# jaidevshriram/loma-nerf

Hardware: AMD Instinct MI355X
Metric: ray-samples/sec fwd+bwd, 4096 rays×64 samples, 1/2/4/8 MI355X (higher is better)
Workload: dtype f32; 1 GPU; cfg3: 4096 rays x 64 samples per GPU, PE F=5, MLP 33->256x7->4, fp32; rays_per_gpu=4096, samples=64, layers=8, width=256, parallelism=dp1, optimizer=adam lr 0.0005 on device (train_nerf.py:133-161), in the step, input=rays: sampling, dists and positional encoding on the GPU

## Files before the change

loma-nerf_amd/csrc/lnerf_dw16.hip:

```cpp
#include "lnerf_internal.h"

namespace lnerf {

namespace {

typedef float fx4 __attribute__((ext_vector_type(4)));
typedef float fx16 __attribute__((ext_vector_type(16)));
typedef __bf16 bf8 __attribute__((ext_vector_type(8)));
typedef __bf16 bf4 __attribute__((ext_vector_type(4)));
typedef _Float16 hf8 __attribute__((ext_vector_type(8)));
typedef _Float16 hf4 __attribute__((ext_vector_type(4)));

#ifndef LNERF_DW16_SPLIT_LATE
#define LNERF_DW16_SPLIT_LATE 1
#endif
#ifndef LNERF_DW16_DEPTH
#define LNERF_DW16_DEPTH 3
#endif

#ifndef LNERF_DW16_XROW
#define LNERF_DW16_XROW 1
#endif

#ifndef LNERF_DW16_WAVES
#define LNERF_DW16_WAVES 8
#endif
constexpr int kWavesDw = LNERF_DW16_WAVES;
static_assert(kWavesDw == 16 || kWavesDw == 8 || kWavesDw == 4, "dW workgroups of 16, 8 or 4 waves");
constexpr int kThreads = 64 * kWavesDw;
// ... 51 lines not shown
__device__ __forceinline__ RowMap row_map(int kt, int nt) {
    RowMap m;
    const int t = threadIdx.x, u = t & 127;
    m.lane = 4 * u;
    m.hstride = 512;
    m.rowo = 16 * ((t >> 6) & 1) + 4 * (t & 3);
    m.isamp = (t & 63) >> 2;
    const int w2 = wave_id() >> 1;
#pragma unroll
    for (int i = 0; i < kRounds; ++i) {
        const int tl = kTileGroups * (i % kRPO) + w2;
        m.ok[i] = tl < (i < kRPO ? kt : nt);
        m.tile[i] = m.ok[i] ? tl : 0;
    }
    return m;
}

__device__ __forceinline__ int image_row(int i, const RowMap& m) {
    return (i < kRPO ? 0 : 256) + 32 * (kTileGroups * (i % kRPO) + (threadIdx.x >> 7)) + m.rowo;
}

struct Loads {
    fx4 v[kRounds];
    unsigned e;
};

__device__ __forceinline__ void sample_shifts(unsigned e, int E, int& ea, int& eg) {
    const int xa = sexp_xa(e), xg = sexp_xg(e);
    if (xa == -128 || xg == -128) {
        ea = xa < -126 ? 0 : xa;
        eg = xg == -128 ? 0 : xg;
        return;
    }
    if (xa == kSexpNonFinite) {
        eg = xg;
        ea = E - xg;
        return;
    }
    const int d = xa + xg - E;
    ea = xa - (d >> 1);
    eg = xg - ((d + 1) >> 1);
}

template <bool A24>
__device__ __forceinline__ void issue_loads(const float* A, const float* G, const unsigned* se, int kt,
                                            int nt, const RowMap& m, int hb, int hb_end, Loads& L) {
    const bool in = hb < hb_end;
    const int hbc = in ? hb : max(0, hb_end - 1);
    L.e = se[hbc * 16 + m.isamp];
    const int blk = hbc >> 1, half = hbc & 1;
    const float* pg = G + (size_t)blk * nt * 1024 + half * m.hstride;
    if constexpr (A24) {
        const unsigned char* pa = (const unsigned char*)A + ((size_t)blk * kt * 3072 + half * 1536 + 12 * (threadIdx.x & 127));
#pragma unroll
        for (int i = 0; i < kRPO; ++i) {
            const unsigned* q = (const unsigned*)(pa + m.tile[i] * 3072);
            L.v[i] = fx4{__builtin_bit_cast(float, __builtin_nontemporal_load(q)),
                         __builtin_bit_cast(float, __builtin_nontemporal_load(q + 1)),
                         __builtin_bit_cast(float, __builtin_nontemporal_load(q + 2)), 0.0f};
        }
    } else {
        const float* pa = A + (size_t)blk * kt * 1024 + half * m.hstride;
#pragma unroll
        for (int i = 0; i < kRPO; ++i) L.v[i] = __builtin_nontemporal_load((const fx4*)(pa + m.tile[i] * 1024 + m.lane));
    }
#pragma unroll
    for (int i = kRPO; i < kRounds; ++i) L.v[i] = __builtin_nontemporal_load((const fx4*)(pg + m.tile[i] * 1024 + m.lane));
}

__device__ __forceinline__ fx4 decode_a24(const fx4& raw) {
    typedef unsigned ux4 __attribute__((ext_vector_type(4)));
    const ux4 d = __builtin_bit_cast(ux4, raw);
    const unsigned d0 = d[0], d1 = d[1], d2 = d[2];
    const unsigned m0 = d0 & 0xFFFFFFu;
    const unsigned m1 = __builtin_amdgcn_alignbit(d1, d0, 24) & 0xFFFFFFu;
    const unsigned m2 = __builtin_amdgcn_alignbit(d2, d1, 16) & 0xFFFFFFu;
    const unsigned m3 = d2 >> 8;
    constexpr float kMagic = 12582912.0f;
    return fx4{__builtin_bit_cast(float, 0x4B000000u | m0) - kMagic, __builtin_bit_cast(float, 0x4B000000u | m1) - kMagic,
               __builtin_bit_cast(float, 0x4B000000u | m2) - kMagic, __builtin_bit_cast(float, 0x4B000000u | m3) - kMagic};
}

__device__ __forceinline__ void split4(const fx4& x, bf4& h, bf4& m, bf4& lo) {
#pragma unroll
    for (int e = 0; e < 4; ++e) {
        const __bf16 hh = (__bf16)x[e];
        const float r = x[e] - (float)hh;
        const __bf16 mm = (__bf16)r;
        h[e] = hh;
        m[e] = mm;
        lo[e] = (__bf16)(r - (float)mm);
    }
}


template <int PL>
__device__ __forceinline__ void write_planes_row(const fx4& v, int i, unsigned char* img, float sa, float sg,
                                                 const RowMap& m) {
    unsigned char* p = img + m.isamp * kImgRow + 8 * ((image_row(i, m) >> 2) ^ swz(m.isamp));
    const float sc = i < kRPO ? sa : sg;
    if constexpr (PL == 2) {
        typedef unsigned u2 __attribute__((ext_vector_type(2)));
        unsigned h0, l0, h1, l1;
        split_h2(v[0], v[1], sc, h0, l0);
        split_h2(v[2], v[3], sc, h1, l1);
        *(u2*)(p) = u2{h0, h1};
        *(u2*)(p + kPlaneBytes) = u2{l0, l1};
    } else if constexpr (PL == 1) {
        const fx4 x = v * sc;
        *(bf4*)(p) = bf4{(__bf16)x[0], (__bf16)x[1], (__bf16)x[2], (__bf16)x[3]};
    } else {
        bf4 h, m, lo;
        split4(v * sc, h, m, lo);
        *(bf4*)(p) = h;
        *(bf4*)(p + kPlaneBytes) = m;
        *(bf4*)(p + 2 * kPlaneBytes) = lo;
    }
}

__device__ __forceinline__ bool xrow(unsigned e, int E) {
    const int xa = sexp_xa(e), xg = sexp_xg(e);
    const int d = xa + xg - E;
    return xa > -127 && xg > -127 && (d < 0 || d > sexp_dmax(e));
}

template <int PL>
__device__ __forceinline__ void sample_scales(unsigned e, int E, float& sa, float& sg) {
    int ea, eg;
    sample_shifts(e, E, ea, eg);
    if constexpr (a24k(PL)) {
        const int xa = sexp_xa(e);
        ea = xa == -128 ? 0 : ea - (xa == kSexpNonFinite ? 0 : xa) - 8;
    }
    sa = __builtin_ldexpf(1.0f, ea);
    sg = __builtin_ldexpf(1.0f, eg);
    if constexpr (PL == 2 && LNERF_DW16_XROW) {
        const bool x = xrow(e, E);
        sa = x ? 0.0f : sa;
        sg = x ? 0.0f : sg;
    }
}

template <int PL>
__device__ __forceinline__ fx4 round_values(const Loads& L, int i) {
    if constexpr (a24k(PL)) {
        if (i >= kRPO) return L.v[i];
        fx4 v = decode_a24(L.v[i]);
        const bool marked = sexp_xa(L.e) == kSexpNonFinite;
        if (__builtin_expect(__builtin_amdgcn_ballot_w64(marked) != 0, 0)) {
#pragma unroll
            for (int j = 0; j < 4; ++j)
                if (marked && __builtin_fabsf(v[j]) >= 4194304.0f) v[j] = __builtin_nanf("");
            asm volatile("" : "+v"(v));
        }
        return v;
    }
    return L.v[i];
}

template <int PL>
__device__ __forceinline__ void write_planes(const Loads& L, unsigned char* img, int E, const RowMap& m) {
    float sa, sg;
    sample_scales<PL>(L.e, E, sa, sg);
#pragma unroll
    for (int i = 0; i < kRounds; ++i) write_planes_row<PL>(round_values<PL>(L, i), i, img, sa, sg, m);
}

__device__ __forceinline__ fx16 mfma32(const bf8& a, const bf8& b, fx16 c) {
    return __builtin_amdgcn_mfma_f32_32x32x16_bf16(a, b, c, 0, 0, 0);
}
__device__ __forceinline__ fx16 mfma32h(const bf8& a, const bf8& b, fx16 c) {
    return __builtin_amdgcn_mfma_f32_32x32x16_f16(__builtin_bit_cast(hf8, a), __builtin_bit_cast(hf8, b), c, 0, 0,
                                                  0);
}

typedef short s4 __attribute__((ext_vector_type(4)));

__device__ __forceinline__ bf8 read_frag(unsigned char* addr) {
    typedef __attribute__((address_space(3))) s4* lp;
    const s4 a = __builtin_amdgcn_ds_read_tr16_b64_v4i16((lp)(__attribute__((address_space(3))) void*)addr);
    const s4 b = __builtin_amdgcn_ds_read_tr16_b64_v4i16(
        (lp)(__attribute__((address_space(3))) void*)(addr + 4 * kImgRow));
    typedef short s8 __attribute__((ext_vector_type(8)));
    return __builtin_bit_cast(bf8, s8{a[0], a[1], a[2], a[3], b[0], b[1], b[2], b[3]});
}

__device__ __forceinline__ int frag_off(int f0) {
    const int l = threadIdx.x & 63;
    const int row = 8 * (l >> 5) + ((l >> 2) & 3);
    const int quad = (f0 >> 2) + 4 * ((l >> 4) & 1) + (l & 3);
    return row * kImgRow + 8 * (quad ^ swz(row));
}

template <int PL>
__device__ __forceinline__ fx16 mma_tile(const bf8 (&ap)[nplanes(PL)], const bf8 (&gp)[nplanes(PL)], fx16 c) {
    if constexpr (PL == 2) {
        c = mfma32h(ap[0], gp[1], c);
        c = mfma32h(ap[1], gp[0], c);
        c = mfma32h(ap[0], gp[0], c);
    } else if constexpr (PL == 1) {
        c = mfma32(ap[0], gp[0], c);
    } else {
        c = mfma32(ap[0], gp[2], c);
        c = mfma32(ap[1], gp[1], c);
        c = mfma32(ap[2], gp[0], c);
        c = mfma32(ap[1], gp[0], c);
        c = mfma32(ap[0], gp[1], c);
        c = mfma32(ap[0], gp[0], c);
    }
    return c;
}

#ifndef LNERF_DW16_PMAJOR
#define LNERF_DW16_PMAJOR 1
#endif
// ... 2 lines not shown
                                        fx16 (&acc)[TI][TJ], int j) {
    if constexpr (!LNERF_DW16_PMAJOR) {
#pragma unroll
        for (int i = 0; i < TI; ++i) acc[i][j] = mma_tile<PL>(ap[i], gp, acc[i][j]);
    } else if constexpr (PL == 2) {
#pragma unroll
        for (int i = 0; i < TI; ++i) acc[i][j] = mfma32h(ap[i][0], gp[1], acc[i][j]);
#pragma unroll
        for (int i = 0; i < TI; ++i) acc[i][j] = mfma32h(ap[i][1], gp[0], acc[i][j]);
#pragma unroll
        for (int i = 0; i < TI; ++i) acc[i][j] = mfma32h(ap[i][0], gp[0], acc[i][j]);
    } else if constexpr (PL == 1) {
#pragma unroll
        for (int i = 0; i < TI; ++i) acc[i][j] = mfma32(ap[i][0], gp[0], acc[i][j]);
    } else {
        constexpr int pa[6] = {0, 1, 2, 1, 0, 0}, pg[6] = {2, 1, 0, 0, 1, 0};
#pragma unroll
        for (int k = 0; k < 6; ++k)
#pragma unroll
            for (int i = 0; i < TI; ++i) acc[i][j] = mfma32(ap[i][pa[k]], gp[pg[k]], acc[i][j]);
    }
}

template <int PL, int TI, int TJ, bool ACTIVE, bool FULL>
__device__ __forceinline__ void block_mma(const unsigned char* img, int a0, int g0, fx16 (&acc)[TI][TJ],
                                          const Loads& nl, unsigned char* nxt, const RowMap& m, int E,
                                          bool live = true) {
    float sa, sg;
    sample_scales<PL>(nl.e, E, sa, sg);
    sa = live ? sa : 0.0f;
    sg = live ? sg : 0.0f;
    const unsigned char* fl = img;
    constexpr int NP = nplanes(PL);
    bf8 ap[TI][NP];
    if constexpr (ACTIVE) {
#pragma unroll
        for (int i = 0; i < TI; ++i)
#pragma unroll
            for (int p = 0; p < NP; ++p) ap[i][p] = read_frag((unsigned char*)fl + p * kPlaneBytes + frag_off(a0 + 32 * i));
    }
    constexpr int RPS = (kWavesDw == 8 || TJ >= kRounds) ? 1 : (kRounds + TJ - 1) / TJ;
    constexpr int NR = (kRounds + RPS - 1) / RPS;
    constexpr int NK = NR > TJ ? NR : TJ;
    auto split = [&](int k) {
#pragma unroll
        for (int r = 0; r < RPS; ++r) {
            const int i = k * RPS + r;
            if (i < kRounds && (FULL || m.ok[i])) write_planes_row<PL>(round_values<PL>(nl, i), i, nxt, sa, sg, m);
        }
    };
#pragma unroll
    for (int k = 0; k < NK; ++k) {
        if (!LNERF_DW16_SPLIT_LATE) split(k);
        if constexpr (ACTIVE) {
            if (k < TJ) {
                const int j = k < TJ ? k : 0;
                bf8 gp[NP];
#pragma unroll
                for (int p = 0; p < NP; ++p) gp[p] = read_frag((unsigned char*)fl + p * kPlaneBytes + frag_off(256 + g0 + 32 * j));
                mma_col<PL, TI, TJ>(ap, gp, acc, j);
            }
        }
        if (LNERF_DW16_SPLIT_LATE) split(k);
    }
}

template <int PL, int TI, int TJ, bool ACTIVE, bool FULL, int I>
__device__ __forceinline__ void hb_step3(const float* A, const float* G, const unsigned* se, int kt, int nt,
                                         const RowMap& m, int hb, int hb0, int hb1, int a0, int g0,
                                         fx16 (&acc)[TI][TJ], Loads& L0, Loads& L1, Loads& L2, fx4 (&dbs)[kRPO],
                                         unsigned char* lds, int E, bool& xany) {
    constexpr int kIB = image_bytes<PL>();
    Loads& fr = I == 0 ? L0 : I == 1 ? L1 : L2;
    const Loads& nx = I == 0 ? L1 : I == 1 ? L2 : L0;
    issue_loads<a24k(PL)>(A, G, se, kt, nt, m, hb + 3, hb1, fr);
    if (hb + 1 < hb1) {
#pragma unroll
        for (int i = 0; i < kRPO; ++i) dbs[i] += nx.v[kRPO + i];
    }
    const int cur = (hb - hb0) & 1;
    block_mma<PL, TI, TJ, ACTIVE, FULL>(lds + cur * kIB, a0, g0, acc, nx, lds + (cur ^ 1) * kIB, m, E, hb + 1 < hb1);
    if constexpr (PL == 2 && LNERF_DW16_XROW) xany |= hb + 1 < hb1 && xrow(nx.e, E);
    __syncthreads();
}

template <int PL, int TI, int TJ, bool ACTIVE, bool FULL>
__device__ __forceinline__ void hb_loop3(const float* A, const float* G, const unsigned* se, int kt, int nt,
                                         const RowMap& m, int hb0, int hb1, int a0, int g0, fx16 (&acc)[TI][TJ],
                                         Loads& L0, Loads& L1, Loads& L2, fx4 (&dbs)[kRPO], unsigned char* lds,
                                         int E, bool& xany) {
    for (int hb = hb0; hb < hb1; hb += 3) {
        hb_step3<PL, TI, TJ, ACTIVE, FULL, 0>(A, G, se, kt, nt, m, hb, hb0, hb1, a0, g0, acc, L0, L1, L2, dbs, lds, E, xany);
        hb_step3<PL, TI, TJ, ACTIVE, FULL, 1>(A, G, se, kt, nt, m, hb + 1, hb0, hb1, a0, g0, acc, L0, L1, L2, dbs, lds, E, xany);
        hb_step3<PL, TI, TJ, ACTIVE, FULL, 2>(A, G, se, kt, nt, m, hb + 2, hb0, hb1, a0, g0, acc, L0, L1, L2, dbs, lds, E, xany);
    }
}

template <int PL, int TI, int TJ, bool ACTIVE, bool FULL, int I>
__device__ __forceinline__ void hb_step2(const float* A, const float* G, const unsigned* se, int kt, int nt,
                                         const RowMap& m, int hb, int hb0, int hb1, int a0, int g0,
                                         fx16 (&acc)[TI][TJ], Loads& L0, Loads& L1, fx4 (&dbs)[kRPO],
                                         unsigned char* lds, int E, bool& xany) {
    constexpr int kIB = image_bytes<PL>();
    Loads& fr = I == 0 ? L0 : L1;
    const Loads& nx = I == 0 ? L1 : L0;
    issue_loads<a24k(PL)>(A, G, se, kt, nt, m, hb + 2, hb1, fr);
    if (hb + 1 < hb1) {
#pragma unroll
        for (int i = 0; i < kRPO; ++i) dbs[i] += nx.v[kRPO + i];
    }
    const int cur = (hb - hb0) & 1;
    block_mma<PL, TI, TJ, ACTIVE, FULL>(lds + cur * kIB, a0, g0, acc, nx, lds + (cur ^ 1) * kIB, m, E, hb + 1 < hb1);
    if constexpr (PL == 2 && LNERF_DW16_XROW) xany |= hb + 1 < hb1 && xrow(nx.e, E);
    __syncthreads();
}

template <int PL, int TI, int TJ, bool ACTIVE, bool FULL>
__device__ __forceinline__ void hb_loop2(const float* A, const float* G, const unsigned* se, int kt, int nt,
                                         const RowMap& m, int hb0, int hb1, int a0, int g0, fx16 (&acc)[TI][TJ],
                                         Loads& L0, Loads& L1, fx4 (&dbs)[kRPO], unsigned char* lds, int E,
                                         bool& xany) {
    for (int hb = hb0; hb < hb1; hb += 2) {
        hb_step2<PL, TI, TJ, ACTIVE, FULL, 0>(A, G, se, kt, nt, m, hb, hb0, hb1, a0, g0, acc, L0, L1, dbs, lds, E, xany);
        hb_step2<PL, TI, TJ, ACTIVE, FULL, 1>(A, G, se, kt, nt, m, hb + 1, hb0, hb1, a0, g0, acc, L0, L1, dbs, lds, E, xany);
    }
}

template <bool A24>
__device__ __forceinline__ void gather_loads(const float* A, const float* G, const unsigned* se, int kt, int nt,
                                             const RowMap& m, int p, Loads& L) {
    const int pc = p < 0 ? 0 : p;
    L.e = se[pc];
    const int hb = pc >> 4, blk = hb >> 1, half = hb & 1;
    const int u = ((int)threadIdx.x & 127 & ~0x3C) | ((pc & 15) << 2);
    const float* pg = G + (size_t)blk * nt * 1024 + half * 512 + 4 * u;
    if constexpr (A24) {
        const unsigned char* pa = (const unsigned char*)A + ((size_t)blk * kt * 3072 + half * 1536 + 12 * u);
#pragma unroll
        for (int i = 0; i < kRPO; ++i) {
            const unsigned* q = (const unsigned*)(pa + m.tile[i] * 3072);
            L.v[i] = fx4{__builtin_bit_cast(float, q[0]), __builtin_bit_cast(float, q[1]),
                         __builtin_bit_cast(float, q[2]), 0.0f};
        }
    } else {
        const float* pa = A + (size_t)blk * kt * 1024 + half * 512 + 4 * u;
#pragma unroll
        for (int i = 0; i < kRPO; ++i) L.v[i] = *(const fx4*)(pa + m.tile[i] * 1024);
    }
#pragma unroll
    for (int i = kRPO; i < kRounds; ++i) L.v[i] = *(const fx4*)(pg + m.tile[i] * 1024);
}

template <int PL, int TI, int TJ>
__device__ __forceinline__ void mma_block(const unsigned char* img, int a0, int g0, fx16 (&acc)[TI][TJ]) {
    constexpr int NP = nplanes(PL);
    bf8 ap[TI][NP];
#pragma unroll
    for (int i = 0; i < TI; ++i)
#pragma unroll
        for (int p = 0; p < NP; ++p) ap[i][p] = read_frag((unsigned char*)img + p * kPlaneBytes + frag_off(a0 + 32 * i));
#pragma unroll
    for (int j = 0; j < TJ; ++j) {
        bf8 gp[NP];
#pragma unroll
        for (int p = 0; p < NP; ++p) gp[p] = read_frag((unsigned char*)img + p * kPlaneBytes + frag_off(256 + g0 + 32 * j));
// ... 58 lines not shown
                ring[(mine + r) % kXrowRing] = base + k * kThreads + tid;
            }
        }
        tail = off;
        __syncthreads();
        const bool last = base + 4 * kThreads >= p1;
        const int ng = last ? (tail - head + 15) / 16 : (tail - head) / 16;
        if (ng > 0) {
            auto pos = [&](int gi) {
                const int at = head + 16 * gi + m.isamp;
                return at < tail ? ring[at % kXrowRing] : -1;
            };
            int pc = pos(0);
            Loads Lc;
            gather_loads<a24k(PX)>(A, G, se, KT, NT, m, pc, Lc);
            for (int gi = 0; gi < ng; ++gi) {
                const int pn = gi + 1 < ng ? pos(gi + 1) : -1;
                Loads Ln;
                if (gi + 1 < ng) gather_loads<a24k(PX)>(A, G, se, KT, NT, m, pn, Ln);
                float sa, sg;
                sample_scales<PX>(Lc.e, E, sa, sg);
                sa = pc < 0 ? 0.0f : sa;
                sg = pc < 0 ? 0.0f : sg;
#pragma unroll
                for (int i = 0; i < kRounds; ++i)
                    if (m.ok[i]) write_planes_row<PX>(round_values<PX>(Lc, i), i, lds, sa, sg, m);
                __syncthreads();
                if (active) mma_block<PX, TI, TJ>(lds, a0, g0, acc);
                __syncthreads();
                Lc = Ln;
                pc = pn;
            }
            head = head + 16 * ng < tail ? head + 16 * ng : tail;
        }
    }
    return int2{tail, ntail};
}

template <int PL, int TI, int TJ>
__device__ __forceinline__ void dw_split(const Dw16Args& a, int l, int sp, unsigned char* lds) {
    const int tid = threadIdx.x, lane = tid & 63, wave = wave_id();
    const int KT = a.kt[l], NT = a.nt[l];
    const int nbg = (NT + TJ - 1) / TJ, nblk = ((KT + TI - 1) / TI) * nbg;
    const bool active = wave < nblk;
    const int a0 = active ? (wave / nbg) * 32 * TI : 0, g0 = active ? (wave % nbg) * 32 * TJ : 0;
    const int hbs = 2 * a.blocks, splits = a.splits[l];
    const int per = (hbs + splits - 1) / splits;
    const int hb0 = min(hbs, sp * per), hb1 = min(hbs, hb0 + per);

    fx16 acc[TI][TJ];
#pragma unroll
    for (int i = 0; i < TI; ++i)
#pragma unroll
        for (int j = 0; j < TJ; ++j) acc[i][j] = fx16{0, 0, 0, 0, 0, 0, 0, 0, 0, 0, 0, 0, 0, 0, 0, 0};
    fx4 dbs[kRPO];
#pragma unroll
    for (int i = 0; i < kRPO; ++i) dbs[i] = fx4{0.0f, 0.0f, 0.0f, 0.0f};

    const float* A = a.act + a.a_off[l];
    const float* G = a.grad + a.g_off[l];
    const RowMap m = row_map(KT, NT);
    const unsigned* se = a.sexp + (size_t)l * a.rpad;
    const int E = a.eshift[l];
    const bool full = KT == 8 && NT == 8;
#if LNERF_DW16_DEPTH == 2
    Loads L0, L1;
    bool xany = false;
    issue_loads<a24k(PL)>(A, G, se, KT, NT, m, hb0, hb1, L0);
    issue_loads<a24k(PL)>(A, G, se, KT, NT, m, hb0 + 1, hb1, L1);
    if (hb0 < hb1) {
#pragma unroll
        for (int i = 0; i < kRPO; ++i) dbs[i] += L0.v[kRPO + i];
        write_planes<PL>(L0, lds, E, m);
        if constexpr (PL == 2 && LNERF_DW16_XROW) xany = xrow(L0.e, E);
    }
    __syncthreads();
    if (active && full) hb_loop2<PL, TI, TJ, true, true>(A, G, se, KT, NT, m, hb0, hb1, a0, g0, acc, L0, L1, dbs, lds, E, xany);
    else if (active) hb_loop2<PL, TI, TJ, true, false>(A, G, se, KT, NT, m, hb0, hb1, a0, g0, acc, L0, L1, dbs, lds, E, xany);
    else if (full) hb_loop2<PL, TI, TJ, false, true>(A, G, se, KT, NT, m, hb0, hb1, a0, g0, acc, L0, L1, dbs, lds, E, xany);
    else hb_loop2<PL, TI, TJ, false, false>(A, G, se, KT, NT, m, hb0, hb1, a0, g0, acc, L0, L1, dbs, lds, E, xany);
#else
    Loads L0, L1, L2;
    bool xany = false;
    issue_loads<a24k(PL)>(A, G, se, KT, NT, m, hb0, hb1, L0);
    issue_loads<a24k(PL)>(A, G, se, KT, NT, m, hb0 + 1, hb1, L1);
    issue_loads<a24k(PL)>(A, G, se, KT, NT, m, hb0 + 2, hb1, L2);
    if (hb0 < hb1) {
#pragma unroll
        for (int i = 0; i < kRPO; ++i) dbs[i] += L0.v[kRPO + i];
        write_planes<PL>(L0, lds, E, m);
        if constexpr (PL == 2 && LNERF_DW16_XROW) xany = xrow(L0.e, E);
    }
    __syncthreads();
    if (active && full) hb_loop3<PL, TI, TJ, true, true>(A, G, se, KT, NT, m, hb0, hb1, a0, g0, acc, L0, L1, L2, dbs, lds, E, xany);
    else if (active) hb_loop3<PL, TI, TJ, true, false>(A, G, se, KT, NT, m, hb0, hb1, a0, g0, acc, L0, L1, L2, dbs, lds, E, xany);
    else if (full) hb_loop3<PL, TI, TJ, false, true>(A, G, se, KT, NT, m, hb0, hb1, a0, g0, acc, L0, L1, L2, dbs, lds, E, xany);
    else hb_loop3<PL, TI, TJ, false, false>(A, G, se, KT, NT, m, hb0, hb1, a0, g0, acc, L0, L1, L2, dbs, lds, E, xany);
#endif

    if constexpr (PL == 2 && LNERF_DW16_XROW) {
        const int2 nx = xrow_pass<TI, TJ>(A, G, se, KT, NT, m, hb0, hb1, a0, g0, active, acc, lds, E, xany);
        if (threadIdx.x == 0 && a.xcount) {
            a.xcount[2 * blockIdx.x] = nx.x;
            a.xcount[2 * blockIdx.x + 1] = nx.y;
        }
    } else {
        if (threadIdx.x == 0 && a.xcount) a.xcount[2 * blockIdx.x] = a.xcount[2 * blockIdx.x + 1] = 0;
    }

    if (active) {
        const int ncol = NT * 32, h = lane >> 5;
        float* part = a.dw_part + a.dwp_off[l] + (size_t)sp * (KT * 32) * ncol;
#pragma unroll
        for (int i = 0; i < TI; ++i)
#pragma unroll
            for (int j = 0; j < TJ; ++j) {
                const int kb = a0 + 32 * i, jb = g0 + 32 * j;
                if (kb < KT * 32 && jb < ncol) {
#pragma unroll
                    for (int r = 0; r < 16; ++r) {
                        const int k = kb + (r & 3) + 8 * (r >> 2) + 4 * h;
// ... 20 lines not shown
}

__host__ __device__ __forceinline__ int dw_shape(int kt, int nt) {
    auto fits = [&](int ti, int tj) { return ((kt + ti - 1) / ti) * ((nt + tj - 1) / tj) <= kWavesDw; };
    if (kWavesDw == 8) {
        if (fits(1, 1)) return 0;
        if (fits(1, 2)) return 1;
        return 2;
    }
    if (kWavesDw == 16) {
        if (fits(1, 1)) return 0;
        if (fits(1, 2)) return 1;
        if (fits(2, 1)) return 3;
        return 4;
    }
    if (fits(1, 1)) return 0;
    if (fits(2, 1)) return 3;
    if (fits(1, 2)) return 1;
    if (fits(2, 2)) return 4;
    return 5;
}

template <int PL>
constexpr int dw_lds_bytes() {
    constexpr int main = 2 * image_bytes<PL>();
    constexpr int xr = PL == 2 && LNERF_DW16_XROW ? image_bytes<kXrowPL>() + (kXrowRing + 9 * kWavesDw) * 4 : 0;
    return main > xr ? main : xr;
}

template <int PL>
__global__ void __launch_bounds__(kThreads, 1) __attribute__((amdgpu_waves_per_eu(kWavesDw / 4, kWavesDw / 4)))
dw16_kernel(Dw16Args a) {
    __shared__ __attribute__((aligned(16))) unsigned char lds[dw_lds_bytes<PL>()];
    if (a.gate && *a.gate == 0) return;
    int li = 0;
    while (li + 1 < a.nl && (int)blockIdx.x >= a.wg_off[li + 1]) ++li;
    const int l = a.lid[li], sp = blockIdx.x - a.wg_off[li];
    if constexpr (kWavesDw == 8) {
        switch (dw_shape(a.kt[l], a.nt[l])) {
            case 0: dw_split<PL, 1, 1>(a, l, sp, lds); break;
            case 1: dw_split<PL, 1, 2>(a, l, sp, lds); break;
            default: dw_split<PL, 2, 4>(a, l, sp, lds); break;
        }
    } else if constexpr (kWavesDw == 16) {
        switch (dw_shape(a.kt[l], a.nt[l])) {
            case 0: dw_split<PL, 1, 1>(a, l, sp, lds); break;
            case 1: dw_split<PL, 1, 2>(a, l, sp, lds); break;
            case 3: dw_split<PL, 2, 1>(a, l, sp, lds); break;
            default: dw_split<PL, 2, 2>(a, l, sp, lds); break;
        }
    } else {
        switch (dw_shape(a.kt[l], a.nt[l])) {
            case 0: dw_split<PL, 1, 1>(a, l, sp, lds); break;
            case 3: dw_split<PL, 2, 1>(a, l, sp, lds); break;
            case 1: dw_split<PL, 1, 2>(a, l, sp, lds); break;
            case 4: dw_split<PL, 2, 2>(a, l, sp, lds); break;
// ... 22 lines not shown
            for (int w = 1; w < 16; ++w) r = min(r, ired[w]);
            eshift[blockIdx.x] = r == (1 << 20) ? 0 : r;
        }
        return;
    }
    float s = 0.0f;
    if (t < 256)
        for (int i = t; i < nwg; i += 256) s += loss_part[i];
    red[t] = s;
    __syncthreads();
    for (int w = 128; w > 0; w >>= 1) {
        if (t < w) red[t] = red[t] + red[t + w];
        __syncthreads();
    }
    if (t == 0) {
        *total = red[0];
        if (out_loss) *out_loss = red[0];
    }
}

}

unsigned dw16_build_knobs() {
    return (LNERF_DW16_SPLIT_LATE != 1 ? kKnobDwSplitLate : 0u) | (LNERF_DW16_DEPTH != 3 ? kKnobDwDepth : 0u) |
           (LNERF_DW16_SWZ != 1 ? kKnobDwSwz : 0u) | (LNERF_A24 != 1 ? kKnobA24 : 0u) |
           (LNERF_DW16_XROW != 1 ? kKnobDwXrow : 0u) |
           (LNERF_DW16_WAVES != 8 || !LNERF_DW16_PMAJOR ? kKnobDwWaves : 0u);
}

void dw16_launch(const FusedPlan& p, hipStream_t s) {
    Dw16Args a{};
    for (int l = 0; l < p.L; ++l) {
        a.kt[l] = p.kt[l];
        a.nt[l] = p.nt[l];
        a.a_off[l] = (l == 0) ? p.x_off : p.act_off[l - 1];
        a.g_off[l] = p.grad_off[l];
        a.splits[l] = p.dw_splits[l];
        a.dwp_off[l] = p.dwp_off[l];
        a.dbp_off[l] = p.dbp_off[l];
        a.lid[l] = l;
        a.wg_off[l] = p.dw_split_off[l];
    }
    a.wg_off[p.L] = p.dw_grid;
    a.nl = p.L;
    a.act = p.act;
    a.grad = p.grad;
    a.blocks = p.blocks;
// ... 22 lines not shown
```

loma-nerf_amd/csrc/lnerf_internal.h:

```cpp
#pragma once

#include <hip/hip_runtime.h>
#include <stddef.h>
#include <stdint.h>

#include "lnerf.h"
#include "lnerf_marshal.h"

namespace lnerf {

constexpr int kWmaxParts = 32;
constexpr int kHeadCols = 16;
constexpr int kDefaultDwGrid = 512;
__host__ __device__ constexpr int default_dw_grid(long long samples) {
    return samples / 128 >= kDefaultDwGrid ? kDefaultDwGrid : samples / 128 <= 256 ? 256 : (int)(samples / 128);
}
constexpr int kXrowD0 = 12;
constexpr int kXrowLast = 127;
__host__ __device__ constexpr int sexp_xa(unsigned e) { return (int)(signed char)(e & 0xFFu); }
__host__ __device__ constexpr int sexp_xg(unsigned e) { return (int)(signed char)((e >> 16) & 0xFFu); }
__host__ __device__ constexpr int sexp_dmax(unsigned e) { return (int)(signed char)(e >> 24); }

__device__ __forceinline__ int fp16x3_shift(float m) {
    if (!(m > 0.0f) || !(m < __builtin_inff())) return 0;
// ... 6 lines not shown
__device__ __forceinline__ void split_h2(float x0, float x1, float sc, unsigned& hi, unsigned& lo) {
    typedef _Float16 h2 __attribute__((ext_vector_type(2)));
    const _Float16 h0 = (_Float16)__builtin_fmaf(x0, sc, 0.0f);
    const _Float16 h1 = (_Float16)__builtin_fmaf(x1, sc, 0.0f);
    const _Float16 l0 = (_Float16)__builtin_fmaf(x0, sc, -(float)h0);
    const _Float16 l1 = (_Float16)__builtin_fmaf(x1, sc, -(float)h1);
    hi = __builtin_bit_cast(unsigned, (h2){h0, h1});
    lo = __builtin_bit_cast(unsigned, (h2){l0, l1});
}

#ifndef LNERF_A24
#define LNERF_A24 1
#endif
__host__ __device__ constexpr bool a24_slabs(int PL) { return PL == 2 && LNERF_A24 != 0; }
constexpr int kSexpNonFinite = -127;
__host__ __device__ constexpr int a_tile_floats(int PL) { return a24_slabs(PL) ? 768 : 1024; }

enum : unsigned {
    kKnobK16FullDma = 1u << 0, kKnobK16KDist = 1u << 1, kKnobK16SplitAt = 1u << 2, kKnobK16Sched = 1u << 3,
    kKnobK16Prio = 1u << 4, kKnobK16Spread = 1u << 5, kKnobProf = 1u << 6, kKnobA24 = 1u << 7,
    kKnobK16Only = 1u << 8, kKnobDwSplitLate = 1u << 9, kKnobDwDepth = 1u << 10, kKnobDwSwz = 1u << 11,
    kKnobK16Pin = 1u << 12, kKnobK16FdSrc = 1u << 13, kKnobKrStagger = 1u << 15, kKnobDwXrow = 1u << 17,
    kKnobGuard = 1u << 25, kKnobK16G2 = 1u << 26, kKnobKrSched = 1u << 18, kKnobDwWaves = 1u << 14, kKnobKrDist = 1u << 19, kKnobPeDoubling = 1u << 20, kKnobK16OneChunk = 1u << 22, kKnobK16WaveComp = 1u << 23, kKnobK16EpiFma = 1u << 24,
};
unsigned k16_build_knobs();
unsigned dw16_build_knobs();
unsigned kr_build_knobs();

__host__ __device__ inline double ray_depth(int j, int S, float near_t, float far_t) {
    if (S <= 1) return (double)near_t;
    if (j == S - 1) return (double)far_t;
    return (double)j * (((double)far_t - (double)near_t) / (double)(S - 1)) + (double)near_t;
}
__host__ __device__ inline float ray_delta(int j, int S, float near_t, float far_t) {
    if (j >= S - 1) return 1e8f;
    return (float)(ray_depth(j + 1, S, near_t, far_t) - ray_depth(j, S, near_t, far_t));
}
__host__ __device__ inline double ray_point(const float* ray6, int c, int j, int S, float near_t,
                                            float far_t) {
    return (double)ray6[c] + (double)ray6[3 + c] * ray_depth(j, S, near_t, far_t);
}


struct LgBuffers {
    const float* X;
    const float* W;
// ... 123 lines not shown
```

Measured before the change: 118.5 million ray-samples/s.

## Precompute per-sample scale table in LDS and interleave dW16 loads with MFMA

The dW16 weight-gradient kernel now precomputes per-sample scale factors into an LDS table in chunks, so the main loop no longer loads and decodes the exponent word every step. Global loads for future blocks are split by round and issued between MFMA columns. A24 activations are read with a single 96-bit buffer load. The G fragment reads are prefetched one column ahead around the fp16 MFMAs, and the LDS addressing is simplified with XOR tile offsets. The aim is to hide load latency and cut scalar and address overhead in the hot loop, at the cost of more LDS, an extra sync per chunk and more register pressure.

```diff
diff --git a/loma-nerf_amd/csrc/lnerf_dw16.hip b/loma-nerf_amd/csrc/lnerf_dw16.hip
--- a/loma-nerf_amd/csrc/lnerf_dw16.hip
+++ b/loma-nerf_amd/csrc/lnerf_dw16.hip
@@ -5,6 +5,7 @@
 namespace {
 
 typedef float fx4 __attribute__((ext_vector_type(4)));
+typedef float fx3 __attribute__((ext_vector_type(3)));
 typedef float fx16 __attribute__((ext_vector_type(16)));
 typedef __bf16 bf8 __attribute__((ext_vector_type(8)));
 typedef __bf16 bf4 __attribute__((ext_vector_type(4)));
@@ -102,55 +103,50 @@
 
 struct Loads {
     fx4 v[kRounds];
+    fx3 a24[kRPO];
     unsigned e;
 };
 
 __device__ __forceinline__ void sample_shifts(unsigned e, int E, int& ea, int& eg) {
     const int xa = sexp_xa(e), xg = sexp_xg(e);
-    if (xa == -128 || xg == -128) {
-        ea = xa < -126 ? 0 : xa;
-        eg = xg == -128 ? 0 : xg;
-        return;
-    }
-    if (xa == kSexpNonFinite) {
-        eg = xg;
-        ea = E - xg;
-        return;
-    }
+    const bool zero = xa == -128 || xg == -128, nonfin = xa == kSexpNonFinite;
     const int d = xa + xg - E;
-    ea = xa - (d >> 1);
-    eg = xg - ((d + 1) >> 1);
-}
-
+    ea = zero ? (xa < -126 ? 0 : xa) : nonfin ? E - xg : xa - (d >> 1);
+    eg = zero ? (xg == -128 ? 0 : xg) : nonfin ? xg : xg - ((d + 1) >> 1);
+}
+
+constexpr int kAllRounds = (1 << kRounds) - 1;
 template <bool A24>
-__device__ __forceinline__ void issue_loads(const float* A, const float* G, const unsigned* se, int kt,
-                                            int nt, const RowMap& m, int hb, int hb_end, Loads& L) {
+__device__ __forceinline__ void issue_loads(const float* A, const float* G, int kt, int nt, const RowMap& m,
+                                            int hb, int hb_end, Loads& L, int rounds = kAllRounds) {
     const bool in = hb < hb_end;
     const int hbc = in ? hb : max(0, hb_end - 1);
-    L.e = se[hbc * 16 + m.isamp];
     const int blk = hbc >> 1, half = hbc & 1;
     const float* pg = G + (size_t)blk * nt * 1024 + half * m.hstride;
-    if constexpr (A24) {
-        const unsigned char* pa = (const unsigned char*)A + ((size_t)blk * kt * 3072 + half * 1536 + 12 * (threadIdx.x & 127));
+    if (!(rounds & ((1 << kRPO) - 1))) {
+    } else if constexpr (A24) {
+        const unsigned char* pa = (const unsigned char*)A + ((size_t)blk * kt * 3072 + half * 1536);
+        const __amdgpu_buffer_rsrc_t rs =
+            __builtin_amdgcn_make_buffer_rsrc((void*)pa, 0, kt * 3072 - 1536, 0x00020000);
 #pragma unroll
         for (int i = 0; i < kRPO; ++i) {
-            const unsigned* q = (const unsigned*)(pa + m.tile[i] * 3072);
-            L.v[i] = fx4{__builtin_bit_cast(float, __builtin_nontemporal_load(q)),
-                         __builtin_bit_cast(float, __builtin_nontemporal_load(q + 1)),
-                         __builtin_bit_cast(float, __builtin_nontemporal_load(q + 2)), 0.0f};
+            if (rounds >> i & 1)
+                L.a24[i] = __builtin_bit_cast(fx3, __builtin_amdgcn_raw_buffer_load_b96(rs, 3 * m.lane, m.tile[i] * 3072, 2));
         }
     } else {
         const float* pa = A + (size_t)blk * kt * 1024 + half * m.hstride;
 #pragma unroll
-        for (int i = 0; i < kRPO; ++i) L.v[i] = __builtin_nontemporal_load((const fx4*)(pa + m.tile[i] * 1024 + m.lane));
-    }
-#pragma unroll
-    for (int i = kRPO; i < kRounds; ++i) L.v[i] = __builtin_nontemporal_load((const fx4*)(pg + m.tile[i] * 1024 + m.lane));
-}
-
-__device__ __forceinline__ fx4 decode_a24(const fx4& raw) {
-    typedef unsigned ux4 __attribute__((ext_vector_type(4)));
-    const ux4 d = __builtin_bit_cast(ux4, raw);
+        for (int i = 0; i < kRPO; ++i)
+            if (rounds >> i & 1) L.v[i] = __builtin_nontemporal_load((const fx4*)(pa + m.tile[i] * 1024 + m.lane));
+    }
+#pragma unroll
+    for (int i = kRPO; i < kRounds; ++i)
+        if (rounds >> i & 1) L.v[i] = __builtin_nontemporal_load((const fx4*)(pg + m.tile[i] * 1024 + m.lane));
+}
+
+__device__ __forceinline__ fx4 decode_a24(const fx3& raw) {
+    typedef unsigned ux3 __attribute__((ext_vector_type(3)));
+    const ux3 d = __builtin_bit_cast(ux3, raw);
     const unsigned d0 = d[0], d1 = d[1], d2 = d[2];
     const unsigned m0 = d0 & 0xFFFFFFu;
     const unsigned m1 = __builtin_amdgcn_alignbit(d1, d0, 24) & 0xFFFFFFu;
@@ -177,7 +173,11 @@
 template <int PL>
 __device__ __forceinline__ void write_planes_row(const fx4& v, int i, unsigned char* img, float sa, float sg,
                                                  const RowMap& m) {
-    unsigned char* p = img + m.isamp * kImgRow + 8 * ((image_row(i, m) >> 2) ^ swz(m.isamp));
+    constexpr bool kRoundConst = kRPO == 1 || kTileGroups % 4 == 0;
+    const int qround = (i < kRPO ? 0 : 64) + 8 * kTileGroups * (i % kRPO);
+    unsigned char* p = kRoundConst
+        ? img + m.isamp * kImgRow + 8 * (((image_row(0, m) >> 2) ^ swz(m.isamp))) + 8 * qround
+        : img + m.isamp * kImgRow + 8 * ((image_row(i, m) >> 2) ^ swz(m.isamp));
     const float sc = i < kRPO ? sa : sg;
     if constexpr (PL == 2) {
         typedef unsigned u2 __attribute__((ext_vector_type(2)));
@@ -221,13 +221,14 @@
     }
 }
 
-template <int PL>
-__device__ __forceinline__ fx4 round_values(const Loads& L, int i) {
+__device__ __forceinline__ bool any_marked(bool marked) { return __builtin_amdgcn_ballot_w64(marked) != 0; }
+
+template <int PL>
+__device__ __forceinline__ fx4 round_values(const Loads& L, int i, bool marked, bool anym) {
     if constexpr (a24k(PL)) {
         if (i >= kRPO) return L.v[i];
-        fx4 v = decode_a24(L.v[i]);
-        const bool marked = sexp_xa(L.e) == kSexpNonFinite;
-        if (__builtin_expect(__builtin_amdgcn_ballot_w64(marked) != 0, 0)) {
+        fx4 v = decode_a24(L.a24[i]);
+        if (__builtin_expect(anym, 0)) {
 #pragma unroll
             for (int j = 0; j < 4; ++j)
                 if (marked && __builtin_fabsf(v[j]) >= 4194304.0f) v[j] = __builtin_nanf("");
@@ -238,12 +239,40 @@
     return L.v[i];
 }
 
-template <int PL>
-__device__ __forceinline__ void write_planes(const Loads& L, unsigned char* img, int E, const RowMap& m) {
+struct SampleScale {
     float sa, sg;
-    sample_scales<PL>(L.e, E, sa, sg);
-#pragma unroll
-    for (int i = 0; i < kRounds; ++i) write_planes_row<PL>(round_values<PL>(L, i), i, img, sa, sg, m);
+    bool marked;
+};
+__device__ __forceinline__ SampleScale decode_scale(const float2& t) {
+    const unsigned b = __builtin_bit_cast(unsigned, t.x);
+    return SampleScale{__builtin_bit_cast(float, b & 0x7FFFFFFFu), t.y, (b >> 31) != 0};
+}
+
+constexpr int kTabPast = 4;
+template <int PL>
+__device__ __forceinline__ bool fill_scales(float2* tab, const unsigned* se, int E, int c0, int c1) {
+    bool x = false;
+    const int n = (c1 - c0 + kTabPast) * 16, nin = (c1 - c0) * 16, last = max(0, c1 - 1) * 16;
+    for (int i = threadIdx.x; i < n; i += kThreads) {
+        const bool in = i < nin;
+        const unsigned e = se[in ? c0 * 16 + i : last + (i & 15)];
+        float sa, sg;
+        sample_scales<PL>(e, E, sa, sg);
+        unsigned ba = in ? __builtin_bit_cast(unsigned, sa) : 0u;
+        if constexpr (a24k(PL)) ba |= sexp_xa(e) == kSexpNonFinite ? 0x80000000u : 0u;
+        if constexpr (PL == 2 && LNERF_DW16_XROW) x |= in && xrow(e, E);
+        tab[i] = float2{__builtin_bit_cast(float, ba), in ? sg : 0.0f};
+    }
+    return x;
+}
+
+template <int PL>
+__device__ __forceinline__ void write_planes(const Loads& L, unsigned char* img, const SampleScale& sc,
+                                             const RowMap& m) {
+    const bool anym = a24k(PL) && any_marked(sc.marked);
+#pragma unroll
+    for (int i = 0; i < kRounds; ++i)
+        write_planes_row<PL>(round_values<PL>(L, i, sc.marked, anym), i, img, sc.sa, sc.sg, m);
 }
 
 __device__ __forceinline__ fx16 mfma32(const bf8& a, const bf8& b, fx16 c) {
@@ -271,6 +300,12 @@
     const int quad = (f0 >> 2) + 4 * ((l >> 4) & 1) + (l & 3);
     return row * kImgRow + 8 * (quad ^ swz(row));
 }
+
+typedef __attribute__((address_space(3))) unsigned char* lds_bytes;
+__device__ __forceinline__ lds_bytes frag_tile(lds_bytes base, int t) {
+    return (lds_bytes)(unsigned long long)((unsigned)(unsigned long long)base ^ (unsigned)(t << 6));
+}
+__device__ __forceinline__ bf8 read_frag(lds_bytes addr) { return read_frag((unsigned char*)addr); }
 
 template <int PL>
 __device__ __forceinline__ fx16 mma_tile(const bf8 (&ap)[nplanes(PL)], const bf8 (&gp)[nplanes(PL)], fx16 c) {
@@ -319,23 +354,38 @@
     }
 }
 
-template <int PL, int TI, int TJ, bool ACTIVE, bool FULL>
+#ifndef LNERF_DW16_AHEAD
+#define LNERF_DW16_AHEAD 1
+#endif
+template <int PL, int TI, int TJ, bool ACTIVE, bool FULL, typename Pre, typename Mid>
 __device__ __forceinline__ void block_mma(const unsigned char* img, int a0, int g0, fx16 (&acc)[TI][TJ],
-                                          const Loads& nl, unsigned char* nxt, const RowMap& m, int E,
-                                          bool live = true) {
-    float sa, sg;
-    sample_scales<PL>(nl.e, E, sa, sg);
-    sa = live ? sa : 0.0f;
-    sg = live ? sg : 0.0f;
+                                          const Loads& nl, unsigned char* nxt, const RowMap& m, Pre&& pre,
+                                          Mid&& mid) {
     const unsigned char* fl = img;
     constexpr int NP = nplanes(PL);
+    constexpr bool AHEAD = LNERF_DW16_AHEAD != 0 && LNERF_DW16_PMAJOR != 0 && PL == 2;
     bf8 ap[TI][NP];
+    static_assert((TI & (TI - 1)) == 0 && (TJ & (TJ - 1)) == 0 && TI <= 4 && TJ <= 4, "frag_tile: aligned tile groups");
+    const lds_bytes fa = (lds_bytes)(__attribute__((address_space(3))) void*)(fl + frag_off(a0));
+    const lds_bytes fg = (lds_bytes)(__attribute__((address_space(3))) void*)(fl + frag_off(256 + g0));
+    bf8 glo, ghi;
+    auto read_g = [&](int j, int p) { return read_frag(frag_tile(fg, j) + p * kPlaneBytes); };
+    SampleScale sc;
+    if constexpr (!AHEAD) sc = pre();
     if constexpr (ACTIVE) {
 #pragma unroll
         for (int i = 0; i < TI; ++i)
 #pragma unroll
-            for (int p = 0; p < NP; ++p) ap[i][p] = read_frag((unsigned char*)fl + p * kPlaneBytes + frag_off(a0 + 32 * i));
-    }
+            for (int p = 0; p < NP; ++p) ap[i][p] = read_frag(frag_tile(fa, i) + p * kPlaneBytes);
+        if constexpr (AHEAD) {
+            glo = read_g(0, 1);
+            ghi = read_g(0, 0);
+            __builtin_amdgcn_sched_barrier(0);
+        }
+    }
+    if constexpr (AHEAD) sc = pre();
+    const float sa = sc.sa, sg = sc.sg;
+    const bool anym = a24k(PL) && any_marked(sc.marked);
     constexpr int RPS = (kWavesDw == 8 || TJ >= kRounds) ? 1 : (kRounds + TJ - 1) / TJ;
     constexpr int NR = (kRounds + RPS - 1) / RPS;
     constexpr int NK = NR > TJ ? NR : TJ;
@@ -343,7 +393,8 @@
 #pragma unroll
         for (int r = 0; r < RPS; ++r) {
             const int i = k * RPS + r;
-            if (i < kRounds && (FULL || m.ok[i])) write_planes_row<PL>(round_values<PL>(nl, i), i, nxt, sa, sg, m);
+            if (i < kRounds && (FULL || m.ok[i]))
+                write_planes_row<PL>(round_values<PL>(nl, i, sc.marked, anym), i, nxt, sa, sg, m);
         }
     };
 #pragma unroll
@@ -352,74 +403,99 @@
         if constexpr (ACTIVE) {
             if (k < TJ) {
                 const int j = k < TJ ? k : 0;
-                bf8 gp[NP];
-#pragma unroll
-                for (int p = 0; p < NP; ++p) gp[p] = read_frag((unsigned char*)fl + p * kPlaneBytes + frag_off(256 + g0 + 32 * j));
-                mma_col<PL, TI, TJ>(ap, gp, acc, j);
+                if constexpr (AHEAD) {
+#pragma unroll
+                    for (int i = 0; i < TI; ++i) acc[i][j] = mfma32h(ap[i][0], glo, acc[i][j]);
+                    if (j + 1 < TJ) {
+                        glo = read_g(j + 1, 1);
+                        __builtin_amdgcn_sched_barrier(0);
+                    }
+#pragma unroll
+                    for (int i = 0; i < TI; ++i) acc[i][j] = mfma32h(ap[i][1], ghi, acc[i][j]);
+#pragma unroll
+                    for (int i = 0; i < TI; ++i) acc[i][j] = mfma32h(ap[i][0], ghi, acc[i][j]);
+                    if (j + 1 < TJ) {
+                        ghi = read_g(j + 1, 0);
+                        __builtin_amdgcn_sched_barrier(0);
+                    }
+                } else {
+                    bf8 gp[NP];
+#pragma unroll
+                    for (int p = 0; p < NP; ++p) gp[p] = read_g(j, p);
+                    mma_col<PL, TI, TJ>(ap, gp, acc, j);
+                }
             }
         }
         if (LNERF_DW16_SPLIT_LATE) split(k);
+        if (k < NR) mid(((1 << RPS) - 1) << (k * RPS) & kAllRounds);
     }
 }
 
 template <int PL, int TI, int TJ, bool ACTIVE, bool FULL, int I>
-__device__ __forceinline__ void hb_step3(const float* A, const float* G, const unsigned* se, int kt, int nt,
+__device__ __forceinline__ void hb_step3(const float* A, const float* G, const float2* tab, int kt, int nt,
                                          const RowMap& m, int hb, int hb0, int hb1, int a0, int g0,
                                          fx16 (&acc)[TI][TJ], Loads& L0, Loads& L1, Loads& L2, fx4 (&dbs)[kRPO],
-                                         unsigned char* lds, int E, bool& xany) {
+                                         unsigned char* lds, float2& scn) {
     constexpr int kIB = image_bytes<PL>();
     Loads& fr = I == 0 ? L0 : I == 1 ? L1 : L2;
     const Loads& nx = I == 0 ? L1 : I == 1 ? L2 : L0;
-    issue_loads<a24k(PL)>(A, G, se, kt, nt, m, hb + 3, hb1, fr);
-    if (hb + 1 < hb1) {
-#pragma unroll
-        for (int i = 0; i < kRPO; ++i) dbs[i] += nx.v[kRPO + i];
-    }
+    auto pre = [&]() {
+        if (hb + 1 < hb1) {
+#pragma unroll
+            for (int i = 0; i < kRPO; ++i) dbs[i] += nx.v[kRPO + i];
+        }
+        const SampleScale sc = decode_scale(scn);
+        scn = tab[(hb + 2 - hb0) * 16];
+        return sc;
+    };
+    auto mid = [&](int rounds) { issue_loads<a24k(PL)>(A, G, kt, nt, m, hb + LNERF_DW16_DEPTH, hb1, fr, rounds); };
     const int cur = (hb - hb0) & 1;
-    block_mma<PL, TI, TJ, ACTIVE, FULL>(lds + cur * kIB, a0, g0, acc, nx, lds + (cur ^ 1) * kIB, m, E, hb + 1 < hb1);
-    if constexpr (PL == 2 && LNERF_DW16_XROW) xany |= hb + 1 < hb1 && xrow(nx.e, E);
+    block_mma<PL, TI, TJ, ACTIVE, FULL>(lds + cur * kIB, a0, g0, acc, nx, lds + (cur ^ 1) * kIB, m, pre, mid);
     __syncthreads();
 }
 
 template <int PL, int TI, int TJ, bool ACTIVE, bool FULL>
-__device__ __forceinline__ void hb_loop3(const float* A, const float* G, const unsigned* se, int kt, int nt,
+__device__ __forceinline__ void hb_loop3(const float* A, const float* G, const float2* tab, int kt, int nt,
                                          const RowMap& m, int hb0, int hb1, int a0, int g0, fx16 (&acc)[TI][TJ],
                                          Loads& L0, Loads& L1, Loads& L2, fx4 (&dbs)[kRPO], unsigned char* lds,
-                                         int E, bool& xany) {
+                                         float2& scn) {
     for (int hb = hb0; hb < hb1; hb += 3) {
-        hb_step3<PL, TI, TJ, ACTIVE, FULL, 0>(A, G, se, kt, nt, m, hb, hb0, hb1, a0, g0, acc, L0, L1, L2, dbs, lds, E, xany);
-        hb_step3<PL, TI, TJ, ACTIVE, FULL, 1>(A, G, se, kt, nt, m, hb + 1, hb0, hb1, a0, g0, acc, L0, L1, L2, dbs, lds, E, xany);
-        hb_step3<PL, TI, TJ, ACTIVE, FULL, 2>(A, G, se, kt, nt, m, hb + 2, hb0, hb1, a0, g0, acc, L0, L1, L2, dbs, lds, E, xany);
+        hb_step3<PL, TI, TJ, ACTIVE, FULL, 0>(A, G, tab, kt, nt, m, hb, hb0, hb1, a0, g0, acc, L0, L1, L2, dbs, lds, scn);
+        hb_step3<PL, TI, TJ, ACTIVE, FULL, 1>(A, G, tab, kt, nt, m, hb + 1, hb0, hb1, a0, g0, acc, L0, L1, L2, dbs, lds, scn);
+        hb_step3<PL, TI, TJ, ACTIVE, FULL, 2>(A, G, tab, kt, nt, m, hb + 2, hb0, hb1, a0, g0, acc, L0, L1, L2, dbs, lds, scn);
     }
 }
 
 template <int PL, int TI, int TJ, bool ACTIVE, bool FULL, int I>
-__device__ __forceinline__ void hb_step2(const float* A, const float* G, const unsigned* se, int kt, int nt,
+__device__ __forceinline__ void hb_step2(const float* A, const float* G, const float2* tab, int kt, int nt,
                                          const RowMap& m, int hb, int hb0, int hb1, int a0, int g0,
                                          fx16 (&acc)[TI][TJ], Loads& L0, Loads& L1, fx4 (&dbs)[kRPO],
-                                         unsigned char* lds, int E, bool& xany) {
+                                         unsigned char* lds, float2& scn) {
     constexpr int kIB = image_bytes<PL>();
     Loads& fr = I == 0 ? L0 : L1;
     const Loads& nx = I == 0 ? L1 : L0;
-    issue_loads<a24k(PL)>(A, G, se, kt, nt, m, hb + 2, hb1, fr);
-    if (hb + 1 < hb1) {
-#pragma unroll
-        for (int i = 0; i < kRPO; ++i) dbs[i] += nx.v[kRPO + i];
-    }
+    auto pre = [&]() {
+        if (hb + 1 < hb1) {
+#pragma unroll
+            for (int i = 0; i < kRPO; ++i) dbs[i] += nx.v[kRPO + i];
+        }
+        const SampleScale sc = decode_scale(scn);
+        scn = tab[(hb + 2 - hb0) * 16];
+        return sc;
+    };
+    auto mid = [&](int rounds) { issue_loads<a24k(PL)>(A, G, kt, nt, m, hb + LNERF_DW16_DEPTH, hb1, fr, rounds); };
     const int cur = (hb - hb0) & 1;
-    block_mma<PL, TI, TJ, ACTIVE, FULL>(lds + cur * kIB, a0, g0, acc, nx, lds + (cur ^ 1) * kIB, m, E, hb + 1 < hb1);
-    if constexpr (PL == 2 && LNERF_DW16_XROW) xany |= hb + 1 < hb1 && xrow(nx.e, E);
+    block_mma<PL, TI, TJ, ACTIVE, FULL>(lds + cur * kIB, a0, g0, acc, nx, lds + (cur ^ 1) * kIB, m, pre, mid);
     __syncthreads();
 }
 
 template <int PL, int TI, int TJ, bool ACTIVE, bool FULL>
-__device__ __forceinline__ void hb_loop2(const float* A, const float* G, const unsigned* se, int kt, int nt,
+__device__ __forceinline__ void hb_loop2(const float* A, const float* G, const float2* tab, int kt, int nt,
                                          const RowMap& m, int hb0, int hb1, int a0, int g0, fx16 (&acc)[TI][TJ],
-                                         Loads& L0, Loads& L1, fx4 (&dbs)[kRPO], unsigned char* lds, int E,
-                                         bool& xany) {
+                                         Loads& L0, Loads& L1, fx4 (&dbs)[kRPO], unsigned char* lds, float2& scn) {
     for (int hb = hb0; hb < hb1; hb += 2) {
-        hb_step2<PL, TI, TJ, ACTIVE, FULL, 0>(A, G, se, kt, nt, m, hb, hb0, hb1, a0, g0, acc, L0, L1, dbs, lds, E, xany);
-        hb_step2<PL, TI, TJ, ACTIVE, FULL, 1>(A, G, se, kt, nt, m, hb + 1, hb0, hb1, a0, g0, acc, L0, L1, dbs, lds, E, xany);
+        hb_step2<PL, TI, TJ, ACTIVE, FULL, 0>(A, G, tab, kt, nt, m, hb, hb0, hb1, a0, g0, acc, L0, L1, dbs, lds, scn);
+        hb_step2<PL, TI, TJ, ACTIVE, FULL, 1>(A, G, tab, kt, nt, m, hb + 1, hb0, hb1, a0, g0, acc, L0, L1, dbs, lds, scn);
     }
 }
 
@@ -436,8 +512,8 @@
 #pragma unroll
         for (int i = 0; i < kRPO; ++i) {
             const unsigned* q = (const unsigned*)(pa + m.tile[i] * 3072);
-            L.v[i] = fx4{__builtin_bit_cast(float, q[0]), __builtin_bit_cast(float, q[1]),
-                         __builtin_bit_cast(float, q[2]), 0.0f};
+            L.a24[i] = fx3{__builtin_bit_cast(float, q[0]), __builtin_bit_cast(float, q[1]),
+                           __builtin_bit_cast(float, q[2])};
         }
     } else {
         const float* pa = A + (size_t)blk * kt * 1024 + half * 512 + 4 * u;
@@ -542,9 +618,10 @@
                 sample_scales<PX>(Lc.e, E, sa, sg);
                 sa = pc < 0 ? 0.0f : sa;
                 sg = pc < 0 ? 0.0f : sg;
+                const bool marked = a24k(PX) && sexp_xa(Lc.e) == kSexpNonFinite, anym = a24k(PX) && any_marked(marked);
 #pragma unroll
                 for (int i = 0; i < kRounds; ++i)
-                    if (m.ok[i]) write_planes_row<PX>(round_values<PX>(Lc, i), i, lds, sa, sg, m);
+                    if (m.ok[i]) write_planes_row<PX>(round_values<PX>(Lc, i, marked, anym), i, lds, sa, sg, m);
                 __syncthreads();
                 if (active) mma_block<PX, TI, TJ>(lds, a0, g0, acc);
                 __syncthreads();
@@ -556,6 +633,20 @@
     }
     return int2{tail, ntail};
 }
+
+template <int PL>
+constexpr int dw_image_bytes() {
+    constexpr int main = 2 * image_bytes<PL>();
+    constexpr int xr = PL == 2 && LNERF_DW16_XROW ? image_bytes<kXrowPL>() + (kXrowRing + 9 * kWavesDw) * 4 : 0;
+    return ((main > xr ? main : xr) + 15) / 16 * 16;
+}
+template <int PL>
+constexpr int dw_chunk_hb() {
+    constexpr int room = (160 * 1024 - dw_image_bytes<PL>()) / (16 * (int)sizeof(float2)) - kTabPast;
+    return (room > 720 ? 720 : room) / 6 * 6;
+}
+template <int PL>
+constexpr int dw_lds_bytes() { return dw_image_bytes<PL>() + (dw_chunk_hb<PL>() + kTabPast) * 16 * (int)sizeof(float2); }
 
 template <int PL, int TI, int TJ>
 __device__ __forceinline__ void dw_split(const Dw16Args& a, int l, int sp, unsigned char* lds) {
@@ -583,40 +674,40 @@
     const unsigned* se = a.sexp + (size_t)l * a.rpad;
     const int E = a.eshift[l];
     const bool full = KT == 8 && NT == 8;
+    float2* tab = (float2*)(lds + dw_image_bytes<PL>());
+    bool xany = false;
+    for (int c0 = hb0; c0 < hb1; c0 += dw_chunk_hb<PL>()) {
+        const int c1 = min(hb1, c0 + dw_chunk_hb<PL>());
+        xany |= fill_scales<PL>(tab, se, E, c0, c1);
+        const float2* tabt = tab + m.isamp;
 #if LNERF_DW16_DEPTH == 2
-    Loads L0, L1;
-    bool xany = false;
-    issue_loads<a24k(PL)>(A, G, se, KT, NT, m, hb0, hb1, L0);
-    issue_loads<a24k(PL)>(A, G, se, KT, NT, m, hb0 + 1, hb1, L1);
-    if (hb0 < hb1) {
+        Loads L0, L1;
+        issue_loads<a24k(PL)>(A, G, KT, NT, m, c0, c1, L0);
+        issue_loads<a24k(PL)>(A, G, KT, NT, m, c0 + 1, c1, L1);
+#else
+        Loads L0, L1, L2;
+        issue_loads<a24k(PL)>(A, G, KT, NT, m, c0, c1, L0);
+        issue_loads<a24k(PL)>(A, G, KT, NT, m, c0 + 1, c1, L1);
+        issue_loads<a24k(PL)>(A, G, KT, NT, m, c0 + 2, c1, L2);
+#endif
+        __syncthreads();
 #pragma unroll
         for (int i = 0; i < kRPO; ++i) dbs[i] += L0.v[kRPO + i];
-        write_planes<PL>(L0, lds, E, m);
-        if constexpr (PL == 2 && LNERF_DW16_XROW) xany = xrow(L0.e, E);
-    }
-    __syncthreads();
-    if (active && full) hb_loop2<PL, TI, TJ, true, true>(A, G, se, KT, NT, m, hb0, hb1, a0, g0, acc, L0, L1, dbs, lds, E, xany);
-    else if (active) hb_loop2<PL, TI, TJ, true, false>(A, G, se, KT, NT, m, hb0, hb1, a0, g0, acc, L0, L1, dbs, lds, E, xany);
-    else if (full) hb_loop2<PL, TI, TJ, false, true>(A, G, se, KT, NT, m, hb0, hb1, a0, g0, acc, L0, L1, dbs, lds, E, xany);
-    else hb_loop2<PL, TI, TJ, false, false>(A, G, se, KT, NT, m, hb0, hb1, a0, g0, acc, L0, L1, dbs, lds, E, xany);
+        write_planes<PL>(L0, lds, decode_scale(tabt[0]), m);
+        float2 scn = tabt[16];
+        __syncthreads();
+#if LNERF_DW16_DEPTH == 2
+        if (active && full) hb_loop2<PL, TI, TJ, true, true>(A, G, tabt, KT, NT, m, c0, c1, a0, g0, acc, L0, L1, dbs, lds, scn);
+        else if (active) hb_loop2<PL, TI, TJ, true, false>(A, G, tabt, KT, NT, m, c0, c1, a0, g0, acc, L0, L1, dbs, lds, scn);
+        else if (full) hb_loop2<PL, TI, TJ, false, true>(A, G, tabt, KT, NT, m, c0, c1, a0, g0, acc, L0, L1, dbs, lds, scn);
+        else hb_loop2<PL, TI, TJ, false, false>(A, G, tabt, KT, NT, m, c0, c1, a0, g0, acc, L0, L1, dbs, lds, scn);
 #else
-    Loads L0, L1, L2;
-    bool xany = false;
-    issue_loads<a24k(PL)>(A, G, se, KT, NT, m, hb0, hb1, L0);
-    issue_loads<a24k(PL)>(A, G, se, KT, NT, m, hb0 + 1, hb1, L1);
-    issue_loads<a24k(PL)>(A, G, se, KT, NT, m, hb0 + 2, hb1, L2);
-    if (hb0 < hb1) {
-#pragma unroll
-        for (int i = 0; i < kRPO; ++i) dbs[i] += L0.v[kRPO + i];
-        write_planes<PL>(L0, lds, E, m);
-        if constexpr (PL == 2 && LNERF_DW16_XROW) xany = xrow(L0.e, E);
-    }
-    __syncthreads();
-    if (active && full) hb_loop3<PL, TI, TJ, true, true>(A, G, se, KT, NT, m, hb0, hb1, a0, g0, acc, L0, L1, L2, dbs, lds, E, xany);
-    else if (active) hb_loop3<PL, TI, TJ, true, false>(A, G, se, KT, NT, m, hb0, hb1, a0, g0, acc, L0, L1, L2, dbs, lds, E, xany);
-    else if (full) hb_loop3<PL, TI, TJ, false, true>(A, G, se, KT, NT, m, hb0, hb1, a0, g0, acc, L0, L1, L2, dbs, lds, E, xany);
-    else hb_loop3<PL, TI, TJ, false, false>(A, G, se, KT, NT, m, hb0, hb1, a0, g0, acc, L0, L1, L2, dbs, lds, E, xany);
+        if (active && full) hb_loop3<PL, TI, TJ, true, true>(A, G, tabt, KT, NT, m, c0, c1, a0, g0, acc, L0, L1, L2, dbs, lds, scn);
+        else if (active) hb_loop3<PL, TI, TJ, true, false>(A, G, tabt, KT, NT, m, c0, c1, a0, g0, acc, L0, L1, L2, dbs, lds, scn);
+        else if (full) hb_loop3<PL, TI, TJ, false, true>(A, G, tabt, KT, NT, m, c0, c1, a0, g0, acc, L0, L1, L2, dbs, lds, scn);
+        else hb_loop3<PL, TI, TJ, false, false>(A, G, tabt, KT, NT, m, c0, c1, a0, g0, acc, L0, L1, L2, dbs, lds, scn);
 #endif
+    }
 
     if constexpr (PL == 2 && LNERF_DW16_XROW) {
         const int2 nx = xrow_pass<TI, TJ>(A, G, se, KT, NT, m, hb0, hb1, a0, g0, active, acc, lds, E, xany);
@@ -683,16 +774,9 @@
 }
 
 template <int PL>
-constexpr int dw_lds_bytes() {
-    constexpr int main = 2 * image_bytes<PL>();
-    constexpr int xr = PL == 2 && LNERF_DW16_XROW ? image_bytes<kXrowPL>() + (kXrowRing + 9 * kWavesDw) * 4 : 0;
-    return main > xr ? main : xr;
-}
-
-template <int PL>
 __global__ void __launch_bounds__(kThreads, 1) __attribute__((amdgpu_waves_per_eu(kWavesDw / 4, kWavesDw / 4)))
 dw16_kernel(Dw16Args a) {
-    __shared__ __attribute__((aligned(16))) unsigned char lds[dw_lds_bytes<PL>()];
+    __shared__ __attribute__((aligned(256))) unsigned char lds[dw_lds_bytes<PL>()];
     if (a.gate && *a.gate == 0) return;
     int li = 0;
     while (li + 1 < a.nl && (int)blockIdx.x >= a.wg_off[li + 1]) ++li;
@@ -761,7 +845,7 @@
 }
 
 unsigned dw16_build_knobs() {
-    return (LNERF_DW16_SPLIT_LATE != 1 ? kKnobDwSplitLate : 0u) | (LNERF_DW16_DEPTH != 3 ? kKnobDwDepth : 0u) |
+    return (LNERF_DW16_SPLIT_LATE != 1 ? kKnobDwSplitLate : 0u) | (LNERF_DW16_AHEAD != 1 ? kKnobDwAhead : 0u) | (LNERF_DW16_DEPTH != 3 ? kKnobDwDepth : 0u) |
            (LNERF_DW16_SWZ != 1 ? kKnobDwSwz : 0u) | (LNERF_A24 != 1 ? kKnobA24 : 0u) |
            (LNERF_DW16_XROW != 1 ? kKnobDwXrow : 0u) |
            (LNERF_DW16_WAVES != 8 || !LNERF_DW16_PMAJOR ? kKnobDwWaves : 0u);
diff --git a/loma-nerf_amd/csrc/lnerf_internal.h b/loma-nerf_amd/csrc/lnerf_internal.h
--- a/loma-nerf_amd/csrc/lnerf_internal.h
+++ b/loma-nerf_amd/csrc/lnerf_internal.h
@@ -52,6 +52,7 @@
     kKnobK16Only = 1u << 8, kKnobDwSplitLate = 1u << 9, kKnobDwDepth = 1u << 10, kKnobDwSwz = 1u << 11,
     kKnobK16Pin = 1u << 12, kKnobK16FdSrc = 1u << 13, kKnobKrStagger = 1u << 15, kKnobDwXrow = 1u << 17,
     kKnobGuard = 1u << 25, kKnobK16G2 = 1u << 26, kKnobKrSched = 1u << 18, kKnobDwWaves = 1u << 14, kKnobKrDist = 1u << 19, kKnobPeDoubling = 1u << 20, kKnobK16OneChunk = 1u << 22, kKnobK16WaveComp = 1u << 23, kKnobK16EpiFma = 1u << 24,
+    kKnobDwAhead = 1u << 27,
 };
 unsigned k16_build_knobs();
 unsigned dw16_build_knobs();
```

Result: faster. 120.8 million ray-samples/s, median of 6 (+2.0%).
